# jgrss/cultionet

Hardware: AMD Instinct MI355X
Metric: train_chips_per_sec (higher is better)
Workload: dtype f32

## Files before the change

### cultionet_amd/csrc/cn_conv.hip

```cpp
#include "cn_common.h"
#include "cn_conv_geom.h"
#include "cn_profile.h"

#include <cstdlib>

#define KC 8

static int cn_reduce_slices(const CnConvGeom& g, hipStream_t stream);

template <int TN, int TM>
__device__ __forceinline__ void cn_igemm_epilogue(const CnConvGeom& g, const f32x16 (&acc)[TN][TM],
                                                  const bool (&pix_ok)[TM], const int (&out_off)[TM], int co_base,
                                                  int half, int grp, int split, int b,
                                                  const float* __restrict__ bias, float* __restrict__ y) {
  const int HWout = g.Hout * g.Wout;
  const bool sliced = g.slice_stride != 0;
  float* yb = sliced ? g.part + (long)(grp * g.splits + split) * g.slice_stride + (long)b * g.Cout * HWout
                     : y + (long)b * g.ybs;
  const bool first = split == 0;
#pragma unroll
  for (int tn = 0; tn < TN; ++tn) {
#pragma unroll
    for (int r = 0; r < 16; ++r) {
      const int co = co_base + tn * 32 + (r & 3) + 8 * (r >> 2) + 4 * half;
// ... 549 lines not shown
  if ((long)g.Cin * g.Hin * g.Win * 4 >= (1L << 31) || (long)(max_taps > 0 ? max_taps : 1) * g.Kpad * g.Npad * 4 >= (1L << 31))
    return CN_ERR_ARG;
  const size_t lds = (size_t)(g.tap_lds_off + 3 * CN_MAX_TAPS + 1) * sizeof(float);
  if (lds > 160 * 1024) return CN_ERR_LDS;
  static bool attr_set = false;
  if (!attr_set) {
    (void)hipFuncSetAttribute((const void*)cn_conv_igemm_kernel<WAVES_N, TN, NI_T>,
                              hipFuncAttributeMaxDynamicSharedMemorySize, 160 * 1024);
    attr_set = true;
  }
  g.grid_x = total_tiles;
  g.grid_y = (g.Cout + NT - 1) / NT;
  g.splits = splits < 1 ? 1 : splits;
  dim3 grid(cn_xcd_grid((long)g.grid_x * g.grid_y * g.splits));
  cn_prof_name("cn_conv_igemm_kernel<%d, %d, %d>", WAVES_N, TN, NI_T);
  cn_prof_desc("igemm_dw<%d,%d,%d> G%d B%d %d->%d %dx%d->%dx%d taps%d cls%d is%d os%d grid%dx%dx%d", WAVES_N, TN, NI_T,
               g.G, g.B, g.Cin, g.Cout, g.Hin, g.Win, g.Hout, g.Wout, max_taps, g.ncls, g.is, g.os, total_tiles,
               (g.Cout + NT - 1) / NT, splits);
  cn_prof_bytes(4.0 * g.G * ((double)g.B * g.Cin * g.Hin * g.Win + (double)g.B * g.Cout * g.Hout * g.Wout / (g.shared_y ? g.G : 1) +
                             (double)(max_taps > 0 ? max_taps : 1) * g.Cin * g.Cout));
  cn_prof_before(stream);
  CN_LAUNCH((cn_conv_igemm_kernel<WAVES_N, TN, NI_T>), grid, dim3(256), lds, stream, g);
  cn_prof_after(stream, NT == 128 ? 0 : 1, flops);
  const int rrc = cn_reduce_slices(g, stream);
  return rrc != CN_OK ? rrc : cn_check_launch();
}

struct CnPlan {
  int total_tiles, max_plane, max_vplane, max_taps;
  int max_rplane, max_absdx;
  double flops;
};

static CnPlan cn_plan(CnConvGeom& g, int MT) {
  CnPlan p = {0, 0, 0, 0, 0, 0, 0.0};
  for (int c = 0; c < g.ncls; ++c) {
    CnConvClass& k = g.cls[c];
    const int Mimg = k.Hg * k.Wg;
    int rows_g = (MT + k.Wg - 2) / k.Wg + 1;
    if (rows_g > k.Hg) rows_g = k.Hg;
    k.min_dy = 0; k.min_dx = 0;
    int max_dy = 0, max_dx = 0;
    for (int t = 0; t < k.ntaps; ++t) {
      if (t == 0 || k.dy[t] < k.min_dy) k.min_dy = k.dy[t];
      if (t == 0 || k.dx[t] < k.min_dx) k.min_dx = k.dx[t];
      if (t == 0 || k.dy[t] > max_dy) max_dy = k.dy[t];
      if (t == 0 || k.dx[t] > max_dx) max_dx = k.dx[t];
    }
    const int rows = (rows_g - 1) * g.is + (max_dy - k.min_dy) + 1;
    k.pitch = (k.Wg - 1) * g.is + (max_dx - k.min_dx) + 1;
    k.plane = rows * k.pitch;
    k.vplane = (rows * g.Win + (max_dx - k.min_dx) + 4 + 3) / 4 * 4;
    k.rows = rows;
    {
      const int rpitch = (g.Win + 3) / 4 * 4 + 4;
      if ((rows + 1) * rpitch + 4 > p.max_rplane) p.max_rplane = (rows + 1) * rpitch + 4;
    }
    if (-k.min_dx > p.max_absdx) p.max_absdx = -k.min_dx;
    if (max_dx > p.max_absdx) p.max_absdx = max_dx;
    k.tiles_per_img = (Mimg + MT - 1) / MT;
    k.block_begin = p.total_tiles;
    p.total_tiles += g.B * k.tiles_per_img;
    if (k.plane > p.max_plane) p.max_plane = k.plane;
    if (k.vplane > p.max_vplane) p.max_vplane = k.vplane;
    if (k.ntaps > p.max_taps) p.max_taps = k.ntaps;
    p.flops += 2.0 * g.B * Mimg * (double)g.Cout * g.Cin * k.ntaps;
  }
  g.interleave = 0;
  if (g.ncls > 1 && g.want_interleave) {
    bool same = true;
    for (int c = 1; c < g.ncls; ++c) same = same && g.cls[c].tiles_per_img == g.cls[0].tiles_per_img;
    g.interleave = same ? 1 : 0;
  }
  return p;
}

struct CnChoice { int cfg, splits, cps; double cost; };

static double cn_launch_cost(long blocks, int cps, double mt_units, int splits, double out_elems) {
  const double F = 273.0, R = 170.0;
  const double c1 = 36.7 + 0.614 * mt_units, c2 = 30.0 + 1.19 * mt_units;
  const long full = blocks / 512, rem = blocks % 512;
  double c = full * (F + cps * c2);
  if (rem > 0) c += F + cps * (rem > 256 ? c2 : c1);
  if (splits > 1) c += R + out_elems * 4.0 * (2.0 * splits + 1.0) / 8.0e6 * (128.0 / 7.5);
  return c;
}

static thread_local float* g_conv_ws;
static thread_local long g_conv_ws_floats;

static CnChoice cn_choose(const CnConvGeom& g0, const int* mts, int ncfg, int NT, bool allow_split) {
  const int nchunks = (g0.Cin + KC - 1) / KC;
  const int ny = (g0.Cout + NT - 1) / NT;
  const int G = g0.G > 0 ? g0.G : 1;
  const double out_elems = (double)g0.B * g0.Cout * g0.Hout * g0.Wout * (g0.shared_y ? 1 : G);
  CnChoice best = {0, 1, nchunks > 0 ? nchunks : 1, 1e300};
  int forced = 0;
  {
    static const char* dbg = getenv("CN_DBG_SPLITS");
    if (dbg) forced = atoi(dbg) < 1 ? 1 : atoi(dbg);
  }
  long ws_cap = 32;
  if (g_conv_ws != nullptr) {
    const long stride = ((long)g0.B * g0.Cout * g0.Hout * g0.Wout + 3) / 4 * 4;
    ws_cap = g_conv_ws_floats / (stride * G);
  }
  int forced_cfg = -1;
  {
    static const char* dbgc = getenv("CN_DBG_CFG");
    if (dbgc) forced_cfg = atoi(dbgc);
  }
  for (int i = 0; i < ncfg; ++i) {
    if (forced_cfg >= 0 && i != (forced_cfg < ncfg ? forced_cfg : ncfg - 1)) continue;
    CnConvGeom gi = g0;
    const CnPlan p = cn_plan(gi, mts[i]);
    if (p.total_tiles <= 0) continue;
    const long base = (long)p.total_tiles * ny;
    int max_splits = (allow_split && p.max_taps > 0 && nchunks >= 4) ? nchunks / 2 : 1;
    if (max_splits > 32) max_splits = 32;
    if (max_splits > ws_cap) max_splits = ws_cap < 1 ? 1 : (int)ws_cap;
    const double taps = p.total_tiles > 0 ? p.flops / (2.0 * g0.Cout * g0.Cin * (double)mts[i] * p.total_tiles) : 9.0;
    const double chunk_units = (double)mts[i] * NT / 128.0 * (taps < 9.0 ? taps : 9.0) / 9.0;
    for (int sp = 1; sp <= max_splits; ++sp) {
      if (forced && sp != (forced > max_splits ? max_splits : forced)) continue;
      const int cps = (nchunks + sp - 1) / sp;
      const int splits = (nchunks + cps - 1) / cps;
      if (splits != sp && !forced) continue;
      const double cost = cn_launch_cost(base * splits, cps, chunk_units, splits, out_elems);
      if (cost < best.cost * (i == best.cfg ? 1.0 : 0.98)) best = {i, splits, cps, cost};
    }
  }
  return best;
}


#include <mutex>
#include <unordered_map>
namespace {
struct CnWs { float* p; long n; };
std::mutex g_ws_mu;
std::unordered_map<void*, CnWs> g_ws_by_stream;
}

extern "C" int cn_conv_set_workspace(void* stream, float* ws, long ws_floats) {
  if (ws != nullptr && ((reinterpret_cast<uintptr_t>(ws) & 15) || ws_floats < 0)) return CN_ERR_ARG;
  std::lock_guard<std::mutex> lk(g_ws_mu);
  if (ws == nullptr) g_ws_by_stream.erase(stream);
  else g_ws_by_stream[stream] = {ws, ws_floats};
  return CN_OK;
}

static void cn_bind_ws(void* stream) {
  std::lock_guard<std::mutex> lk(g_ws_mu);
  auto it = g_ws_by_stream.find(stream);
  if (it == g_ws_by_stream.end()) { g_conv_ws = nullptr; g_conv_ws_floats = 0; }
  else { g_conv_ws = it->second.p; g_conv_ws_floats = it->second.n; }
}

struct CnReduceArgs {
  const float* part;
  long slice_stride;
  int nsum;
  int ngrp;
  float* y[CN_MAX_GROUPS];
  const float* bias[CN_MAX_GROUPS * CN_MAX_GROUPS];
  int nbias;
  long ybs;
  int B, Cout, HW, accumulate;
};

__global__ __launch_bounds__(256) void cn_conv_reduce_kernel(const CnReduceArgs a) {
  const long n = (long)a.Cout * a.HW;
  const int b = blockIdx.y, gi = blockIdx.z;
  const float* p0 = a.part + (long)gi * a.nsum * a.slice_stride + (long)b * n;
  float* yb = a.y[gi] + (long)b * a.ybs;
  for (long i = (blockIdx.x * 256L + threadIdx.x) * 4; i < n; i += (long)gridDim.x * 1024) {
    if (i + 3 < n && (n & 3) == 0 && (a.ybs & 3) == 0 && (reinterpret_cast<uintptr_t>(yb) & 15) == 0) {
      f32x4 s = *reinterpret_cast<const f32x4*>(p0 + i);
      for (int k = 1; k < a.nsum; ++k) s += *reinterpret_cast<const f32x4*>(p0 + (long)k * a.slice_stride + i);
#pragma unroll
      for (int e = 0; e < 4; ++e) {
        const int c = (int)((i + e) / a.HW);
        for (int j = 0; j < a.nbias; ++j)
          if (a.bias[gi * CN_MAX_GROUPS + j] != nullptr) s[e] += a.bias[gi * CN_MAX_GROUPS + j][c];
      }
      f32x4* d = reinterpret_cast<f32x4*>(yb + i);
      *d = a.accumulate ? *d + s : s;
    } else {
      for (long e = i; e < n && e < i + 4; ++e) {
        float s = p0[e];
        for (int k = 1; k < a.nsum; ++k) s += p0[(long)k * a.slice_stride + e];
        const int c = (int)(e / a.HW);
        for (int j = 0; j < a.nbias; ++j)
          if (a.bias[gi * CN_MAX_GROUPS + j] != nullptr) s += a.bias[gi * CN_MAX_GROUPS + j][c];
        yb[e] = a.accumulate ? yb[e] + s : s;
      }
    }
  }
}

static int cn_finish_split(CnConvGeom& g, const CnPlan& p, int splits, int cps, float* y, hipStream_t stream) {
  (void)y;
  const int nchunks = (g.Cin + KC - 1) / KC;
  g.chunks_per_split = cps > 0 ? cps : (nchunks > 0 ? nchunks : 1);
  if (p.max_taps == 0) g.chunks_per_split = nchunks > 0 ? nchunks : 1;
  g.splits = splits < 1 ? 1 : splits;
  g.atomic_out = g.splits > 1 || (g.G > 1 && g.shared_y);
  g.part = nullptr;
  g.slice_stride = 0;
  if (g.atomic_out) {
    const long stride = ((long)g.B * g.Cout * g.Hout * g.Wout + 3) / 4 * 4;
    if (g_conv_ws != nullptr && stride * g.G * g.splits <= g_conv_ws_floats) {
      g.part = g_conv_ws;
      g.slice_stride = stride;
      return CN_OK;
    }
  }
  if (g.atomic_out && !g.accumulate) {
    const int ny = g.shared_y ? 1 : g.G;
    for (int i = 0; i < ny; ++i)
      if (hipMemsetAsync(g.gy[i], 0, sizeof(float) * (size_t)g.B * g.Cout * g.Hout * g.Wout, stream) != hipSuccess)
        return CN_ERR_LAUNCH;
  }
  return CN_OK;
}

static int cn_reduce_slices(const CnConvGeom& g, hipStream_t stream) {
  if (g.slice_stride == 0) return CN_OK;
  CnReduceArgs a = {};
  a.part = g.part;
  a.slice_stride = g.slice_stride;
  a.ybs = g.ybs; a.B = g.B; a.Cout = g.Cout; a.HW = g.Hout * g.Wout; a.accumulate = g.accumulate;
  if (g.shared_y) {
    a.nsum = g.G * g.splits; a.ngrp = 1; a.y[0] = g.gy[0]; a.nbias = g.G;
    for (int j = 0; j < g.G; ++j) a.bias[j] = g.gbias[j];
  } else {
    a.nsum = g.splits; a.ngrp = g.G; a.nbias = 1;
    for (int i = 0; i < g.G; ++i) { a.y[i] = g.gy[i]; a.bias[i * CN_MAX_GROUPS] = g.gbias[i]; }
  }
  const long n = (long)g.Cout * a.HW;
  long bx = (n + 1023) / 1024;
  if (bx > 1024) bx = 1024;
  CN_LAUNCH(cn_conv_reduce_kernel, dim3((unsigned)bx, g.B, a.ngrp), dim3(256), 0, stream, a);
  return cn_check_launch();
}

template <int WAVES_N, int TN, int TM>
static int cn_launch_vec_cfg(const float* x, const float* wp, const float* bias, float* y, CnConvGeom& g, int splits,
                             int cps, hipStream_t stream) {
  constexpr int MT = (4 / WAVES_N) * TM * 32;
  const CnPlan p = cn_plan(g, MT);
  if (p.total_tiles <= 0) return CN_OK;
  const int rp = g.odd_planes ? 3
                 : (p.max_rplane <= 4096 && p.max_absdx <= 4) ? (g.Win % 4 == 0 ? 1 : (g.Win % 2 == 0 ? 2 : 0)) : 0;
  const int img = (rp == 1 || rp == 2) ? p.max_rplane : p.max_vplane;
  g.w_lds_off = KC * 1024 * (img <= 1024 ? 1 : (img <= 2048 ? 2 : 4)) + (rp == 3 ? 16 : 0);
  const int rc = cn_finish_split(g, p, splits, cps, y, stream);
  if (rc != CN_OK) return rc;
#define CN_GO(NV_, RP_) \
  return cn_launch_igemm_v<WAVES_N, TN, TM, NV_, RP_>(x, wp, bias, y, g, p.total_tiles, p.max_taps, splits, p.flops, stream)
  if (rp == 1) {
    if (img <= 1024) CN_GO(1, 1);
    if (img <= 2048) CN_GO(2, 1);
    CN_GO(4, 1);
  }
  if (rp == 2) {
    if (img <= 1024) CN_GO(1, 2);
    if (img <= 2048) CN_GO(2, 2);
    CN_GO(4, 2);
  }
  if (rp == 3) {
    if (img <= 1024) CN_GO(1, 3);
    if (img <= 2048) CN_GO(2, 3);
    CN_GO(4, 3);
  }
  if (img <= 1024) CN_GO(1, 0);
  if (img <= 2048) CN_GO(2, 0);
  CN_GO(4, 0);
#undef CN_GO
}

template <int WAVES_N, int TN>
static int cn_launch_dword_cfg(const float* x, const float* wp, const float* bias, float* y, CnConvGeom& g,
                               int splits, int cps, hipStream_t stream) {
  constexpr int MT = (4 / WAVES_N) * 64;
  const CnPlan p = cn_plan(g, MT);
  if (p.total_tiles <= 0) return CN_OK;
  if (p.max_plane > 12 * 256) return CN_ERR_LDS;
  g.w_lds_off = (KC * p.max_plane + 3) / 4 * 4;
  const int rc = cn_finish_split(g, p, splits, cps, y, stream);
  if (rc != CN_OK) return rc;
  if (p.max_plane <= 3 * 256)
    return cn_launch_igemm_t<WAVES_N, TN, 3>(x, wp, bias, y, g, p.total_tiles, p.max_taps, splits, p.flops, stream);
  if (p.max_plane <= 6 * 256)
    return cn_launch_igemm_t<WAVES_N, TN, 6>(x, wp, bias, y, g, p.total_tiles, p.max_taps, splits, p.flops, stream);
  return cn_launch_igemm_t<WAVES_N, TN, 12>(x, wp, bias, y, g, p.total_tiles, p.max_taps, splits, p.flops, stream);
}

struct CnGemm1x1 {
  int B, Cin, Cout, HW, Kpad, Npad, tiles_per_img, grid_x, grid_y, accumulate;
  long xbs, ybs;
};
#define KC1 32

template <int TM>
__global__ __launch_bounds__(256) void cn_conv1x1_kernel(const float* __restrict__ x, const float* __restrict__ wp,
                                                        const float* __restrict__ bias, float* __restrict__ y,
                                                        const CnGemm1x1 g) {
  constexpr int MT = TM * 32, NT = 128;
  constexpr int NA = KC1 * NT / 4 / 256;
  constexpr int NB = (KC1 * MT / 4 + 255) / 256;
  __shared__ __attribute__((aligned(16))) float a_lds[KC1 * NT];
  __shared__ __attribute__((aligned(16))) float b_lds[KC1 * MT];
  int bx, by, bz;
  if (!cn_xcd_block(g.grid_x, g.grid_y, g.grid_x * g.grid_y, bx, by, bz)) return;
  const int tid = threadIdx.x, lane = tid & 63, wn = tid >> 6;
  const int half = lane >> 5, l31 = lane & 31;
  const int b = bx / g.tiles_per_img;
  const int p0 = (bx - b * g.tiles_per_img) * MT;
  const int n0 = by * NT;
  const float* xb = x + (long)b * g.xbs;

  f32x16 acc[TM];
#pragma unroll
  for (int tm = 0; tm < TM; ++tm)
#pragma unroll
    for (int r = 0; r < 16; ++r) acc[tm][r] = 0.f;

  f32x4 ra[NA], rb[NB];
  const f32x4 zero4 = {0.f, 0.f, 0.f, 0.f};
#define CN_G1_PREFETCH(c0_)                                                                          \
  {                                                                                                  \
    const int c0 = (c0_);                                                                            \
    _Pragma("unroll") for (int k = 0; k < NA; ++k) {                                                 \
      const int i = tid + k * 256, row = i / (NT / 4), c4 = i - row * (NT / 4);                      \
      ra[k] = (c0 + row) < g.Kpad                                                                    \
                  ? *reinterpret_cast<const f32x4*>(wp + (long)(c0 + row) * g.Npad + n0 + c4 * 4)    \
                  : zero4;                                                                           \
    }                                                                                                \
    _Pragma("unroll") for (int k = 0; k < NB; ++k) {                                                 \
      const int i = tid + k * 256, row = i / (MT / 4), q = i - row * (MT / 4);                       \
      const int p = p0 + q * 4;                                                                      \
      rb[k] = (i < KC1 * MT / 4 && (c0 + row) < g.Cin && p < g.HW)                                   \
                  ? *reinterpret_cast<const f32x4*>(xb + (long)(c0 + row) * g.HW + p)                \
                  : zero4;                                                                           \
    }                                                                                                \
  }
  const int nchunks = (g.Cin + KC1 - 1) / KC1;
  CN_G1_PREFETCH(0);
  for (int ch = 0; ch < nchunks; ++ch) {
    __syncthreads();
#pragma unroll
    for (int k = 0; k < NA; ++k) *reinterpret_cast<f32x4*>(a_lds + (tid + k * 256) * 4) = ra[k];
#pragma unroll
    for (int k = 0; k < NB; ++k)
      if (tid + k * 256 < KC1 * MT / 4) *reinterpret_cast<f32x4*>(b_lds + (tid + k * 256) * 4) = rb[k];
    __syncthreads();
    if (ch + 1 < nchunks) CN_G1_PREFETCH((ch + 1) * KC1);
    const float* ap = a_lds + half * NT + wn * 32 + l31;
    const float* bp = b_lds + half * MT + l31;
#pragma unroll
    for (int k2 = 0; k2 < KC1 / 2; ++k2) {
      const float av = ap[k2 * 2 * NT];
#pragma unroll
      for (int tm = 0; tm < TM; ++tm)
        acc[tm] = __builtin_amdgcn_mfma_f32_32x32x2f32(av, bp[k2 * 2 * MT + tm * 32], acc[tm], 0, 0, 0);
    }
  }
#undef CN_G1_PREFETCH
  float* yb = y + (long)b * g.ybs;
#pragma unroll
  for (int r = 0; r < 16; ++r) {
    const int co = n0 + wn * 32 + (r & 3) + 8 * (r >> 2) + 4 * half;
    if (co < g.Cout) {
      const float bv = bias != nullptr ? bias[co] : 0.f;
#pragma unroll
      for (int tm = 0; tm < TM; ++tm) {
        const int p = p0 + tm * 32 + l31;
        if (p < g.HW) {
          float* dst = yb + (long)co * g.HW + p;
          const float v = acc[tm][r] + bv;
          *dst = g.accumulate ? *dst + v : v;
        }
      }
    }
  }
}

static int cn_conv1x1_launch(const float* x, long xbs, const float* wp, const float* bias, float* y, long ybs, int B,
                             int Cin, int HW, int Cout, int accumulate, hipStream_t stream) {
  if ((HW & 3) || (xbs & 3) || (reinterpret_cast<uintptr_t>(x) & 15)) return CN_ERR_ARG;
  CnGemm1x1 g = {};
  g.B = B; g.Cin = Cin; g.Cout = Cout; g.HW = HW; g.xbs = xbs; g.ybs = ybs; g.accumulate = accumulate;
  g.Kpad = cn_conv_kpad(Cin);
  g.Npad = cn_conv_npad(Cout);
  if (cn_pick_nt(Cout) != 128) return CN_ERR_ARG;
  g.grid_y = (Cout + 127) / 128;
  const long t160 = (long)B * ((HW + 159) / 160) * g.grid_y, t128 = (long)B * ((HW + 127) / 128) * g.grid_y;
  const bool use160 = ((t160 + 511) / 512) * 160 <= ((t128 + 511) / 512) * 128;
  const long blocks = use160 ? t160 : t128;
  if (blocks < 256) return CN_ERR_ARG;
  g.tiles_per_img = use160 ? (HW + 159) / 160 : (HW + 127) / 128;
  g.grid_x = B * g.tiles_per_img;
  const double flops = 2.0 * B * HW * (double)Cout * Cin;
  cn_prof_name("cn_conv1x1_kernel<%d>", use160 ? 5 : 4);
  cn_prof_desc("gemm1x1<%d> B%d %d->%d HW%d grid%dx%d", use160 ? 5 : 4, B, Cin, Cout, HW, g.grid_x, g.grid_y);
  cn_prof_before(stream);
  if (use160)
    CN_LAUNCH((cn_conv1x1_kernel<5>), dim3(cn_xcd_grid(blocks)), dim3(256), 0, stream, x, wp, bias, y, g);
  else
    CN_LAUNCH((cn_conv1x1_kernel<4>), dim3(cn_xcd_grid(blocks)), dim3(256), 0, stream, x, wp, bias, y, g);
  cn_prof_after(stream, 0, flops);
  return cn_check_launch();
}

#include <functional>
static int g_autotune = 0;
static std::unordered_map<uint64_t, CnChoice> g_tuned;
static std::mutex g_tune_mu;

extern "C" int cn_conv_set_autotune(int on) {
  std::lock_guard<std::mutex> lk(g_tune_mu);
  g_autotune = on ? 1 : 0;
  if (!on) g_tuned.clear();
  return CN_OK;
}

static uint64_t cn_tune_key(const CnConvGeom& g, bool vec, int nt, bool allow_split) {
  uint64_t h = 1469598103934665603ull;
  auto mix = [&](long v) { h = (h ^ (uint64_t)v) * 1099511628211ull; };
  mix(g.B); mix(g.Cin); mix(g.Hin); mix(g.Win); mix(g.Cout); mix(g.Hout); mix(g.Wout); mix(g.is); mix(g.os);
  mix(g.ncls); mix(g.G); mix(g.shared_y); mix(vec); mix(nt); mix(allow_split); mix(g_conv_ws != nullptr);
  for (int c = 0; c < g.ncls; ++c) {
    const CnConvClass& k = g.cls[c];
    mix(k.Hg); mix(k.Wg); mix(k.ntaps); mix(k.grp);
    for (int t = 0; t < k.ntaps; ++t) { mix(k.dy[t]); mix(k.dx[t]); }
  }
  return h;
}

static CnChoice cn_autotune(const CnConvGeom& g, const int* mts, int ncfg, int nt, bool allow_split,
                            const CnChoice& model, const std::function<int(const CnChoice&, CnConvGeom&)>& run,
                            hipStream_t stream) {
  static const int split_set[] = {1, 2, 3, 4, 6, 8, 12, 16, 24, 32};
  const int nchunks = (g.Cin + KC - 1) / KC;
  const int ny = (g.Cout + nt - 1) / nt;
  long ws_cap = 32;
  if (g_conv_ws != nullptr) {
    const long stride = ((long)g.B * g.Cout * g.Hout * g.Wout + 3) / 4 * 4;
    ws_cap = g_conv_ws_floats / (stride * (g.G > 0 ? g.G : 1));
  }
  hipEvent_t e0, e1;
  if (hipEventCreate(&e0) != hipSuccess || hipEventCreate(&e1) != hipSuccess) return model;
  CnChoice best = model;
  float best_ms = 1e30f;
  for (int i = 0; i < ncfg; ++i) {
    CnConvGeom gi = g;
    const CnPlan p = cn_plan(gi, mts[i]);
    if (p.total_tiles <= 0) continue;
    int max_splits = (allow_split && p.max_taps > 0 && nchunks >= 4) ? nchunks / 2 : 1;
    if (max_splits > 32) max_splits = 32;
    if (max_splits > ws_cap) max_splits = ws_cap < 1 ? 1 : (int)ws_cap;
    for (int sp : split_set) {
      if (sp > max_splits) break;
      const int cps = (nchunks + sp - 1) / sp;
      const int splits = (nchunks + cps - 1) / cps;
      if (splits != sp) continue;
      if ((long)p.total_tiles * ny * splits > 8192) continue;
      const CnChoice c = {i, splits, cps, 0.0};
      float ms = 0.f;
      bool ok = true;
      for (int rep = 0; rep < 2 && ok; ++rep) {
        CnConvGeom gg = g;
        ok = hipEventRecord(e0, stream) == hipSuccess && run(c, gg) == CN_OK &&
             hipEventRecord(e1, stream) == hipSuccess && hipEventSynchronize(e1) == hipSuccess &&
             hipEventElapsedTime(&ms, e0, e1) == hipSuccess;
      }
      if (ok && ms < best_ms) { best_ms = ms; best = c; }
    }
  }
  (void)hipEventDestroy(e0);
  (void)hipEventDestroy(e1);
  return best;
}

int cn_conv_igemm_launch(CnConvGeom& g, hipStream_t stream) {
  if (g.ncls < 1 || g.ncls > CN_MAX_CLASSES || g.B <= 0 || g.G < 1) return g.B <= 0 ? CN_OK : CN_ERR_ARG;
  g.splits = 1;
  const float* x = g.gx[0]; const float* wp = g.gwp[0]; const float* bias = g.gbias[0]; float* y = g.gy[0];
  g.Kpad = cn_conv_kpad(g.Cin);
  g.Npad = cn_conv_npad(g.Cout);
  const int nt = cn_pick_nt(g.Cout);
  const bool dense_out = g.ybs == (long)g.Cout * g.Hout * g.Wout;
  const bool ws_fits = g_conv_ws != nullptr &&
                       (((long)g.B * g.Cout * g.Hout * g.Wout + 3) / 4 * 4) * g.G * 32 <= g_conv_ws_floats;
  const bool allow_split = dense_out || g.accumulate || ws_fits;
  if (g.G > 1 && g.shared_y && !allow_split) return CN_ERR_ARG;
  const int hw4 = (int)(((long)g.Hin * g.Win) % 4);
  g.odd_planes = (hw4 == 1 && !(g.is > 1 && (long)g.Hin * g.Win > 4096)) ? 1 : 0;
  bool vec = (hw4 == 0 || g.odd_planes) && (g.xbs % 4 == 0);
  if (g.is > 1 && (long)g.Hin * g.Win > 4096) vec = false;
  if ((long)g.Cin * g.Hin * g.Win * 4 >= (1L << 31) || (long)CN_MAX_TAPS * cn_conv_kpad(g.Cin) * g.Npad * 4 >= (1L << 31))
    return CN_ERR_ARG;
  for (int i = 0; i < g.G; ++i) vec = vec && ((reinterpret_cast<uintptr_t>(g.gx[i]) & 15) == 0);
  if (vec) {
    CnConvGeom t = g;
    vec = cn_plan(t, 256).max_vplane <= 4 * 1024;
  }
  static const int mts128[3] = {128, 96, 160};
  static const int mts128d[1] = {128};
  static const int mts256[1] = {256};
  const int* mts = nt == 128 ? (vec ? mts128 : mts128d) : mts256;
  const int ncfg = (nt == 128 && vec) ? 3 : 1;
  auto run = [&](const CnChoice& c, CnConvGeom& gg) -> int {
    if (nt == 128) {
      if (vec) {
        switch (c.cfg) {
          case 1: return cn_launch_vec_cfg<4, 1, 3>(x, wp, bias, y, gg, c.splits, c.cps, stream);
          case 2: return cn_launch_vec_cfg<4, 1, 5>(x, wp, bias, y, gg, c.splits, c.cps, stream);
          default: return cn_launch_vec_cfg<2, 2, 2>(x, wp, bias, y, gg, c.splits, c.cps, stream);
        }
      }
      return cn_launch_dword_cfg<2, 2>(x, wp, bias, y, gg, c.splits, c.cps, stream);
    }
    int rc;
    if (nt == 64) {
      if (vec) return cn_launch_vec_cfg<1, 2, 2>(x, wp, bias, y, gg, c.splits, c.cps, stream);
      rc = cn_launch_dword_cfg<1, 2>(x, wp, bias, y, gg, c.splits, c.cps, stream);
    } else {
      if (vec) return cn_launch_vec_cfg<1, 1, 2>(x, wp, bias, y, gg, c.splits, c.cps, stream);
      rc = cn_launch_dword_cfg<1, 1>(x, wp, bias, y, gg, c.splits, c.cps, stream);
    }
    if (rc == CN_ERR_LDS) {
      CnConvGeom g2 = gg;
      rc = cn_launch_dword_cfg<2, 2>(x, wp, bias, y, g2, c.splits, c.cps, stream);
    }
    return rc;
  };
  CnChoice c = cn_choose(g, mts, ncfg, nt, allow_split);
  if (g_autotune) {
    std::lock_guard<std::mutex> lk(g_tune_mu);
    const uint64_t key = cn_tune_key(g, vec, nt, allow_split);
    auto it = g_tuned.find(key);
    if (it != g_tuned.end()) {
      c = it->second;
    } else if (!g.accumulate && !cn_prof_on()) {
      c = cn_autotune(g, mts, ncfg, nt, allow_split, c, run, stream);
      g_tuned.emplace(key, c);
    }
  }
  return run(c, g);
}

static int cn_set_groups(CnConvGeom& g, int G, const float* const* xs, const float* const* wps,
                         const float* const* biases, float* const* ys) {
  if (G < 1 || G > CN_MAX_GROUPS) return CN_ERR_ARG;
  g.G = G;
  int same = 0;
  for (int i = 0; i < G; ++i) {
    g.gx[i] = xs[i]; g.gwp[i] = wps[i]; g.gbias[i] = biases ? biases[i] : nullptr; g.gy[i] = ys[i];
    if (ys[i] == ys[0]) ++same;
  }
  if (same != G && same != 1) return CN_ERR_ARG;
  for (int i = 1; i < G && same == 1; ++i)
    for (int j = 1; j < i; ++j)
      if (ys[i] == ys[j]) return CN_ERR_ARG;
  g.shared_y = (G > 1 && same == G) ? 1 : 0;
  g.has_bias = 0;
  for (int i = 0; i < G; ++i) g.has_bias |= g.gbias[i] != nullptr;
  return CN_OK;
}

static int cn_gather_conv_g(int G, const float* const* xs, long xbs, const float* const* wps,
                            const float* const* biases, float* const* ys, long ybs, int B, int Cin, int Hin,
                            int Win, int Cout, int Hout, int Wout, int KH, int KW, int stride, const int* pads,
                            const int* dils, int accumulate, hipStream_t stream) {
  if (KH * KW > CN_MAX_TAPS || stride < 1) return CN_ERR_ARG;
  if (Hout <= 0 || Wout <= 0) return CN_OK;
  if (G == 1 && KH == 1 && KW == 1 && stride == 1 && pads[0] == 0 && Hout == Hin && Wout == Win) {
    const int r1 = cn_conv1x1_launch(xs[0], xbs, wps[0], biases ? biases[0] : nullptr, ys[0], ybs, B, Cin, Hin * Win,
                                     Cout, accumulate, stream);
    if (r1 != CN_ERR_ARG) return r1;
  }
  CnConvGeom g = {};
  const int rc = cn_set_groups(g, G, xs, wps, biases, ys);
  if (rc != CN_OK) return rc;
  g.B = B; g.Cin = Cin; g.Hin = Hin; g.Win = Win; g.Cout = Cout; g.Hout = Hout; g.Wout = Wout;
  g.xbs = xbs; g.ybs = ybs; g.is = stride; g.os = 1;
  g.ncls = G;
  for (int i = 0; i < G; ++i) {
    if (dils[i] < 1) return CN_ERR_ARG;
    CnConvClass& k = g.cls[i];
    k.grp = i;
    k.Hg = Hout; k.Wg = Wout; k.oy0 = 0; k.ox0 = 0;
    k.ntaps = cn_gather_taps(KH, KW, pads[i], dils[i], k.dy, k.dx, k.wt);
  }
  g.accumulate = accumulate;
  return cn_conv_igemm_launch(g, stream);
}

static int cn_gather_conv(const float* x, long xbs, const float* wp, const float* bias, float* y, long ybs, int B,
                          int Cin, int Hin, int Win, int Cout, int Hout, int Wout, int KH, int KW, int stride,
                          int pad, int dil, int accumulate, hipStream_t stream) {
  return cn_gather_conv_g(1, &x, xbs, &wp, &bias, &y, ybs, B, Cin, Hin, Win, Cout, Hout, Wout, KH, KW, stride, &pad,
                          &dil, accumulate, stream);
}

extern "C" int cn_conv2d_fwd_f32(const float* x, long xbs, const float* wp, const float* bias, float* y,
                                 long ybs, int B, int Cin, int Hin, int Win, int Cout, int KH, int KW,
                                 int stride, int pad, int dil, int accumulate, void* stream) {
  cn_bind_ws(stream);
  if (stride < 1) return CN_ERR_ARG;
  const int Hout = cn_conv_out(Hin, KH, stride, pad, dil);
  const int Wout = cn_conv_out(Win, KW, stride, pad, dil);
  return cn_gather_conv(x, xbs, wp, bias, y, ybs, B, Cin, Hin, Win, Cout, Hout, Wout, KH, KW, stride, pad, dil,
                        accumulate, (hipStream_t)stream);
}

static int cn_scatter_conv_g(int G, const float* const* srcs, long sbs, const float* const* wps,
                             const float* const* biases, float* const* outs, long obs, int B, int Csrc, int Hs,
                             int Ws, int Cdst, int Ho, int Wo, const int* khs, const int* kws, int stride,
                             const int* pads, const int* dils, int accumulate, hipStream_t stream) {
  if (stride < 1 || G * stride * stride > CN_MAX_CLASSES) return CN_ERR_ARG;
  for (int i = 0; i < G; ++i)
    if (khs[i] * kws[i] > CN_MAX_TAPS || khs[i] < 1 || kws[i] < 1) return CN_ERR_ARG;
  if (G == 1 && khs[0] == 1 && kws[0] == 1 && stride == 1 && pads[0] == 0 && Ho == Hs && Wo == Ws) {
    const int r1 = cn_conv1x1_launch(srcs[0], sbs, wps[0], biases ? biases[0] : nullptr, outs[0], obs, B, Csrc,
                                     Hs * Ws, Cdst, accumulate, stream);
    if (r1 != CN_ERR_ARG) return r1;
  }
  CnConvGeom g = {};
  const int rc = cn_set_groups(g, G, srcs, wps, biases, outs);
  if (rc != CN_OK) return rc;
  g.B = B; g.Cin = Csrc; g.Hin = Hs; g.Win = Ws; g.Cout = Cdst; g.Hout = Ho; g.Wout = Wo;
  g.xbs = sbs; g.ybs = obs; g.is = 1; g.os = stride;
  g.accumulate = accumulate;
  int nc = 0;
  for (int gi = 0; gi < G; ++gi) {
    const int pad = pads[gi], dil = dils[gi], KH = khs[gi], KW = kws[gi];
    if (dil < 1) return CN_ERR_ARG;
    for (int py = 0; py < stride; ++py)
      for (int px = 0; px < stride; ++px) {
        CnConvClass& k = g.cls[nc];
        k.grp = gi;
        k.Hg = cn_parity_extent(Ho, py, stride);
        k.Wg = cn_parity_extent(Wo, px, stride);
        if (k.Hg <= 0 || k.Wg <= 0) continue;
        k.oy0 = py; k.ox0 = px;
        k.ntaps = cn_parity_taps(py, px, KH, KW, stride, pad, dil, k.dy, k.dx, k.wt);
        ++nc;
      }
  }
  g.ncls = nc;
  if (nc == 0) return CN_OK;
  cn_sort_heavy_first(g.cls, nc);
  g.want_interleave = stride > 1 ? 1 : 0;
  return cn_conv_igemm_launch(g, stream);
}

static int cn_scatter_conv(const float* src, long sbs, const float* wp, const float* bias, float* out, long obs,
                           int B, int Csrc, int Hs, int Ws, int Cdst, int Ho, int Wo, int KH, int KW,
                           int stride, int pad, int dil, int accumulate, hipStream_t stream) {
  return cn_scatter_conv_g(1, &src, sbs, &wp, &bias, &out, obs, B, Csrc, Hs, Ws, Cdst, Ho, Wo, &KH, &KW, stride, &pad,
                           &dil, accumulate, stream);
}

extern "C" int cn_conv2d_bwd_data_f32(const float* dy, long dybs, const float* wp_t, float* dx, long dxbs,
                                      int B, int Cin, int Hin, int Win, int Cout, int KH, int KW, int stride,
                                      int pad, int dil, int accumulate, void* stream) {
  cn_bind_ws(stream);
  if (stride < 1) return CN_ERR_ARG;
  const int Hout = cn_conv_out(Hin, KH, stride, pad, dil);
  const int Wout = cn_conv_out(Win, KW, stride, pad, dil);
  return cn_scatter_conv(dy, dybs, wp_t, nullptr, dx, dxbs, B, Cout, Hout, Wout, Cin, Hin, Win, KH, KW, stride,
                         pad, dil, accumulate, (hipStream_t)stream);
}

extern "C" int cn_conv2d_fwd_grouped_f32(int G, const float* const* xs, long xbs, const float* const* wps,
                                         const float* const* biases, float* const* ys, long ybs, int B, int Cin,
                                         int Hin, int Win, int Cout, int KH, int KW, int stride, const int* pads,
                                         const int* dils, int accumulate, void* stream) {
  cn_bind_ws(stream);
  if (G < 1 || G > CN_MAX_GROUPS) return CN_ERR_ARG;
  if (stride < 1) return CN_ERR_ARG;
  const int Hout = cn_conv_out(Hin, KH, stride, pads[0], dils[0]);
  const int Wout = cn_conv_out(Win, KW, stride, pads[0], dils[0]);
  for (int i = 1; i < G; ++i)
    if (cn_conv_out(Hin, KH, stride, pads[i], dils[i]) != Hout ||
        cn_conv_out(Win, KW, stride, pads[i], dils[i]) != Wout)
      return CN_ERR_ARG;
  return cn_gather_conv_g(G, xs, xbs, wps, biases, ys, ybs, B, Cin, Hin, Win, Cout, Hout, Wout, KH, KW, stride,
                          pads, dils, accumulate, (hipStream_t)stream);
}

extern "C" int cn_conv2d_bwd_data_grouped_f32(int G, const float* const* dys, long dybs, const float* const* wps_t,
                                              float* const* dxs, long dxbs, int B, int Cin, int Hin, int Win,
                                              int Cout, const int* khs, const int* kws, int stride, const int* pads,
                                              const int* dils, int accumulate, void* stream) {
  cn_bind_ws(stream);
  if (G < 1 || G > CN_MAX_GROUPS) return CN_ERR_ARG;
  if (stride < 1) return CN_ERR_ARG;
  const int Hout = cn_conv_out(Hin, khs[0], stride, pads[0], dils[0]);
  const int Wout = cn_conv_out(Win, kws[0], stride, pads[0], dils[0]);
  for (int i = 1; i < G; ++i)
    if (cn_conv_out(Hin, khs[i], stride, pads[i], dils[i]) != Hout ||
        cn_conv_out(Win, kws[i], stride, pads[i], dils[i]) != Wout)
      return CN_ERR_ARG;
  return cn_scatter_conv_g(G, dys, dybs, wps_t, nullptr, dxs, dxbs, B, Cout, Hout, Wout, Cin, Hin, Win, khs, kws,
                           stride, pads, dils, accumulate, (hipStream_t)stream);
}

extern "C" int cn_conv_transpose2d_fwd_f32(const float* x, long xbs, const float* wp, const float* bias,
                                           float* y, long ybs, int B, int Cin, int Hin, int Win, int Cout,
                                           int KH, int KW, int stride, int pad, int out_pad, int accumulate,
                                           void* stream) {
  cn_bind_ws(stream);
// ... 70 lines not shown
```

Before: 385.0.

## Rewrite 1x1 conv GEMM with direct global-to-LDS DMA multi-stage pipeline

Replaces the register-staged 1x1 conv GEMM with a templated kernel that copies weight and activation tiles straight into LDS through global_load_lds, using an NST-deep buffer ring synchronised by explicit vmcnt waits and barriers. It adds odd-HW and dword-aligned staging variants plus smaller tile configurations chosen by a cost heuristic, so shapes that earlier returned an argument error (unaligned HW, Cout not suited to 128-wide tiles, too few blocks) now run on the GEMM path. The goal is to hide global load latency, drop the register round-trip, and cover more layers. In exchange it relies on hand-written inline waitcnt asm and dynamic LDS sizing, and the odd-HW path uses skewed indexing that is easy to get wrong.

```diff
diff --git a/cultionet_amd/csrc/cn_conv.hip b/cultionet_amd/csrc/cn_conv.hip
--- a/cultionet_amd/csrc/cn_conv.hip
+++ b/cultionet_amd/csrc/cn_conv.hip
@@ -875,73 +875,134 @@
   int B, Cin, Cout, HW, Kpad, Npad, tiles_per_img, grid_x, grid_y, accumulate;
   long xbs, ybs;
 };
-#define KC1 32
-
-template <int TM>
-__global__ __launch_bounds__(256) void cn_conv1x1_kernel(const float* __restrict__ x, const float* __restrict__ wp,
-                                                        const float* __restrict__ bias, float* __restrict__ y,
-                                                        const CnGemm1x1 g) {
-  constexpr int MT = TM * 32, NT = 128;
-  constexpr int NA = KC1 * NT / 4 / 256;
-  constexpr int NB = (KC1 * MT / 4 + 255) / 256;
-  __shared__ __attribute__((aligned(16))) float a_lds[KC1 * NT];
-  __shared__ __attribute__((aligned(16))) float b_lds[KC1 * MT];
+#define CN_G1_ALIGNED 0
+#define CN_G1_ODD 1
+#define CN_G1_DWORD 2
+
+typedef __attribute__((address_space(3))) void* cn_g1_lds_ptr;
+typedef const __attribute__((address_space(1))) void* cn_g1_gbl_ptr;
+static __device__ float cn_g1_zero[256];
+
+template <int BYTES>
+__device__ __forceinline__ void cn_g1_glds(const float* src, float* lds_wave_base) {
+  if constexpr (BYTES == 16)
+    __builtin_amdgcn_global_load_lds((cn_g1_gbl_ptr)src, (cn_g1_lds_ptr)lds_wave_base, 16, 0, 0);
+  else
+    __builtin_amdgcn_global_load_lds((cn_g1_gbl_ptr)src, (cn_g1_lds_ptr)lds_wave_base, 4, 0, 0);
+}
+
+template <int WN, int WM, int TM, int KCH, int STG, int NST>
+struct CnG1Cfg {
+  static constexpr int NW = WN * WM, NT = WN * 32, MT = WM * TM * 32;
+  static constexpr int VB = STG == CN_G1_DWORD ? 4 : 16;
+  static constexpr int MTP = MT + (STG == CN_G1_ODD ? 4 : 0);
+  static constexpr int BPI = VB == 16 ? 256 : 64;
+  static constexpr int NBI = (KCH * MTP + BPI - 1) / BPI;
+  static constexpr int BIMG = NBI * BPI;
+  static constexpr int AIMG = KCH * NT;
+  static constexpr size_t LDS = sizeof(float) * NST * (AIMG + BIMG);
+};
+
+template <int WN, int WM, int TM, int KCH, int STG, int NST>
+__global__ __launch_bounds__(64 * WN * WM) void cn_gemm1x1_kernel(const float* __restrict__ x,
+                                                                  const float* __restrict__ wp,
+                                                                  const float* __restrict__ bias,
+                                                                  float* __restrict__ y, const CnGemm1x1 g) {
+  using C = CnG1Cfg<WN, WM, TM, KCH, STG, NST>;
+  constexpr int NW = C::NW, NT = C::NT, MT = C::MT, VB = C::VB, MTP = C::MTP, BPI = C::BPI, NBI = C::NBI;
+  constexpr int BIMG = C::BIMG, AIMG = C::AIMG;
+  constexpr int NA = AIMG / 256 / NW;
+  constexpr int NBW = (NBI + NW - 1) / NW;
+  constexpr bool ODD = STG == CN_G1_ODD;
+  static_assert(AIMG % (256 * NW) == 0, "a weight chunk is a whole number of DMA instructions per wave");
+  static_assert(STG != CN_G1_DWORD || (MT & (MT - 1)) == 0, "the dword variant decodes pixels with shifts");
+  constexpr int INFL = (NST - 2) * (NA + NBI / NW);
+  static_assert(NST >= 2 && INFL < 64, "vmcnt is a 6-bit counter");
+  extern __shared__ __attribute__((aligned(16))) float smem[];
+  float* a_lds = smem;
+  float* b_lds = smem + NST * AIMG;
+
   int bx, by, bz;
   if (!cn_xcd_block(g.grid_x, g.grid_y, g.grid_x * g.grid_y, bx, by, bz)) return;
-  const int tid = threadIdx.x, lane = tid & 63, wn = tid >> 6;
+  const int tid = threadIdx.x, lane = tid & 63;
+  const int wid = __builtin_amdgcn_readfirstlane(tid >> 6);
   const int half = lane >> 5, l31 = lane & 31;
+  const int wn = wid % WN, wm = wid / WN;
   const int b = bx / g.tiles_per_img;
   const int p0 = (bx - b * g.tiles_per_img) * MT;
+  const float* xb = x + (long)b * g.xbs;
+  const float* zero16 = cn_g1_zero + 4 * lane;
+  const float* zerob = cn_g1_zero + (VB == 16 ? 4 : 1) * lane;
+  const int nch = (g.Cin + KCH - 1) / KCH;
+  const long img = (long)g.Cin * g.HW;
+
   const int n0 = by * NT;
-  const float* xb = x + (long)b * g.xbs;
+  auto stage_a = [&](int c0, int buf) {
+    float* dst = a_lds + buf * AIMG;
+#pragma unroll
+    for (int k = 0; k < NA; ++k) {
+      const int inst = wid + NW * k;
+      const int p = inst * 64 + lane;
+      const int row = c0 + p / (NT / 4), c4 = p % (NT / 4);
+      const float* src = row < g.Kpad ? wp + (long)row * g.Npad + n0 + 4 * c4 : zero16;
+      cn_g1_glds<16>(src, dst + inst * 256);
+    }
+  };
+  auto stage_b = [&](int c0, int buf) {
+    float* dst = b_lds + buf * BIMG;
+#pragma unroll
+    for (int k = 0; k < NBW; ++k) {
+      const int inst = wid + NW * k;
+      if (NBI % NW == 0 || inst < NBI) {
+        const int e = inst * BPI + (VB == 16 ? 4 : 1) * lane;
+        const int r = e / MTP, row = c0 + r;
+        const int pix = p0 + e % MTP - (ODD ? (row & 3) : 0);
+        const long f = (long)row * g.HW + pix;
+        bool ok = r < KCH && row < g.Cin && pix < g.HW;
+        if (ODD) ok = ok && f + 3 < img;
+        const float* src = ok ? xb + f : zerob;
+        cn_g1_glds<VB>(src, dst + inst * BPI);
+      }
+    }
+  };
 
   f32x16 acc[TM];
 #pragma unroll
   for (int tm = 0; tm < TM; ++tm)
 #pragma unroll
     for (int r = 0; r < 16; ++r) acc[tm][r] = 0.f;
-
-  f32x4 ra[NA], rb[NB];
-  const f32x4 zero4 = {0.f, 0.f, 0.f, 0.f};
-#define CN_G1_PREFETCH(c0_)                                                                          \
-  {                                                                                                  \
-    const int c0 = (c0_);                                                                            \
-    _Pragma("unroll") for (int k = 0; k < NA; ++k) {                                                 \
-      const int i = tid + k * 256, row = i / (NT / 4), c4 = i - row * (NT / 4);                      \
-      ra[k] = (c0 + row) < g.Kpad                                                                    \
-                  ? *reinterpret_cast<const f32x4*>(wp + (long)(c0 + row) * g.Npad + n0 + c4 * 4)    \
-                  : zero4;                                                                           \
-    }                                                                                                \
-    _Pragma("unroll") for (int k = 0; k < NB; ++k) {                                                 \
-      const int i = tid + k * 256, row = i / (MT / 4), q = i - row * (MT / 4);                       \
-      const int p = p0 + q * 4;                                                                      \
-      rb[k] = (i < KC1 * MT / 4 && (c0 + row) < g.Cin && p < g.HW)                                   \
-                  ? *reinterpret_cast<const f32x4*>(xb + (long)(c0 + row) * g.HW + p)                \
-                  : zero4;                                                                           \
-    }                                                                                                \
-  }
-  const int nchunks = (g.Cin + KC1 - 1) / KC1;
-  CN_G1_PREFETCH(0);
-  for (int ch = 0; ch < nchunks; ++ch) {
-    __syncthreads();
-#pragma unroll
-    for (int k = 0; k < NA; ++k) *reinterpret_cast<f32x4*>(a_lds + (tid + k * 256) * 4) = ra[k];
-#pragma unroll
-    for (int k = 0; k < NB; ++k)
-      if (tid + k * 256 < KC1 * MT / 4) *reinterpret_cast<f32x4*>(b_lds + (tid + k * 256) * 4) = rb[k];
-    __syncthreads();
-    if (ch + 1 < nchunks) CN_G1_PREFETCH((ch + 1) * KC1);
-    const float* ap = a_lds + half * NT + wn * 32 + l31;
-    const float* bp = b_lds + half * MT + l31;
-#pragma unroll
-    for (int k2 = 0; k2 < KC1 / 2; ++k2) {
+  auto compute = [&](int buf) {
+    const float* ap = a_lds + buf * AIMG + half * NT + wn * 32 + l31;
+    const float* bp = b_lds + buf * BIMG + half * (MTP + (ODD ? 1 : 0)) + wm * (TM * 32) + l31;
+#pragma unroll
+    for (int k2 = 0; k2 < KCH / 2; ++k2) {
       const float av = ap[k2 * 2 * NT];
 #pragma unroll
       for (int tm = 0; tm < TM; ++tm)
-        acc[tm] = __builtin_amdgcn_mfma_f32_32x32x2f32(av, bp[k2 * 2 * MT + tm * 32], acc[tm], 0, 0, 0);
-    }
-  }
-#undef CN_G1_PREFETCH
+        acc[tm] = __builtin_amdgcn_mfma_f32_32x32x2f32(av, bp[k2 * 2 * MTP + (ODD ? (2 * k2) & 3 : 0) + tm * 32], acc[tm],
+                                                       0, 0, 0);
+    }
+  };
+#pragma unroll
+  for (int s = 0; s < NST - 1; ++s)
+    if (s < nch) {
+      stage_a(s * KCH, s);
+      stage_b(s * KCH, s);
+    }
+  int buf = 0, nbuf = NST - 1;
+  for (int ch = 0; ch < nch; ++ch) {
+    if (ch + NST - 1 <= nch)
+      asm volatile("s_waitcnt vmcnt(%0) lgkmcnt(0)\n\ts_barrier" ::"n"(INFL) : "memory");
+    else
+      asm volatile("s_waitcnt vmcnt(0) lgkmcnt(0)\n\ts_barrier" ::: "memory");
+    if (ch + NST - 1 < nch) {
+      stage_a((ch + NST - 1) * KCH, nbuf);
+      stage_b((ch + NST - 1) * KCH, nbuf);
+    }
+    compute(buf);
+    buf = buf + 1 == NST ? 0 : buf + 1;
+    nbuf = nbuf + 1 == NST ? 0 : nbuf + 1;
+  }
   float* yb = y + (long)b * g.ybs;
 #pragma unroll
   for (int r = 0; r < 16; ++r) {
@@ -950,7 +1011,7 @@
       const float bv = bias != nullptr ? bias[co] : 0.f;
 #pragma unroll
       for (int tm = 0; tm < TM; ++tm) {
-        const int p = p0 + tm * 32 + l31;
+        const int p = p0 + wm * (TM * 32) + tm * 32 + l31;
         if (p < g.HW) {
           float* dst = yb + (long)co * g.HW + p;
           const float v = acc[tm][r] + bv;
@@ -961,31 +1022,66 @@
   }
 }
 
+template <int WN, int WM, int TM, int KCH, int STG, int NST>
+static int cn_gemm1x1_go(const float* x, const float* wp, const float* bias, float* y, CnGemm1x1& g,
+                         hipStream_t stream) {
+  using C = CnG1Cfg<WN, WM, TM, KCH, STG, NST>;
+  g.tiles_per_img = (g.HW + C::MT - 1) / C::MT;
+  g.grid_x = g.B * g.tiles_per_img;
+  g.grid_y = (g.Cout + C::NT - 1) / C::NT;
+  constexpr size_t lds = C::LDS;
+  static_assert(lds <= 160 * 1024, "LDS of one CU");
+  static bool attr_set = false;
+  if (!attr_set) {
+    (void)hipFuncSetAttribute((const void*)cn_gemm1x1_kernel<WN, WM, TM, KCH, STG, NST>,
+                              hipFuncAttributeMaxDynamicSharedMemorySize, 160 * 1024);
+    attr_set = true;
+  }
+  const double flops = 2.0 * g.B * g.HW * (double)g.Cout * g.Cin;
+  cn_prof_name("cn_gemm1x1_kernel<%d, %d, %d, %d, %d, %d>", WN, WM, TM, KCH, STG, NST);
+  cn_prof_desc("gemm1x1<%dx%d,k%dx%d,%s> B%d %d->%d HW%d grid%dx%d", C::NT, C::MT, KCH, NST,
+               STG == CN_G1_ALIGNED ? "v16" : (STG == CN_G1_ODD ? "odd16" : "v4"), g.B, g.Cin, g.Cout, g.HW, g.grid_x,
+               g.grid_y);
+  cn_prof_before(stream);
+  CN_LAUNCH((cn_gemm1x1_kernel<WN, WM, TM, KCH, STG, NST>), dim3(cn_xcd_grid((long)g.grid_x * g.grid_y)),
+            dim3(64 * WN * WM), lds, stream, x, wp, bias, y, g);
+  cn_prof_after(stream, 0, flops);
+  return cn_check_launch();
+}
+
 static int cn_conv1x1_launch(const float* x, long xbs, const float* wp, const float* bias, float* y, long ybs, int B,
                              int Cin, int HW, int Cout, int accumulate, hipStream_t stream) {
-  if ((HW & 3) || (xbs & 3) || (reinterpret_cast<uintptr_t>(x) & 15)) return CN_ERR_ARG;
+  if (B <= 0 || Cin <= 0 || Cout <= 0 || HW <= 0) return CN_ERR_ARG;
+  if (reinterpret_cast<uintptr_t>(wp) & 15) return CN_ERR_ARG;
   CnGemm1x1 g = {};
   g.B = B; g.Cin = Cin; g.Cout = Cout; g.HW = HW; g.xbs = xbs; g.ybs = ybs; g.accumulate = accumulate;
   g.Kpad = cn_conv_kpad(Cin);
   g.Npad = cn_conv_npad(Cout);
-  if (cn_pick_nt(Cout) != 128) return CN_ERR_ARG;
-  g.grid_y = (Cout + 127) / 128;
-  const long t160 = (long)B * ((HW + 159) / 160) * g.grid_y, t128 = (long)B * ((HW + 127) / 128) * g.grid_y;
-  const bool use160 = ((t160 + 511) / 512) * 160 <= ((t128 + 511) / 512) * 128;
-  const long blocks = use160 ? t160 : t128;
-  if (blocks < 256) return CN_ERR_ARG;
-  g.tiles_per_img = use160 ? (HW + 159) / 160 : (HW + 127) / 128;
-  g.grid_x = B * g.tiles_per_img;
-  const double flops = 2.0 * B * HW * (double)Cout * Cin;
-  cn_prof_name("cn_conv1x1_kernel<%d>", use160 ? 5 : 4);
-  cn_prof_desc("gemm1x1<%d> B%d %d->%d HW%d grid%dx%d", use160 ? 5 : 4, B, Cin, Cout, HW, g.grid_x, g.grid_y);
-  cn_prof_before(stream);
-  if (use160)
-    CN_LAUNCH((cn_conv1x1_kernel<5>), dim3(cn_xcd_grid(blocks)), dim3(256), 0, stream, x, wp, bias, y, g);
-  else
-    CN_LAUNCH((cn_conv1x1_kernel<4>), dim3(cn_xcd_grid(blocks)), dim3(256), 0, stream, x, wp, bias, y, g);
-  cn_prof_after(stream, 0, flops);
-  return cn_check_launch();
+  const bool img16 = !(xbs & 3) && !(reinterpret_cast<uintptr_t>(x) & 15);
+  const int stg = (img16 && (HW & 3) == 0) ? CN_G1_ALIGNED
+                  : (img16 && (HW & 3) == 1 && (Cin & 3) == 0) ? CN_G1_ODD : CN_G1_DWORD;
+  const int nt = cn_pick_nt(Cout);
+  auto blocks = [&](int ntile, int mtile) {
+    return (long)B * ((HW + mtile - 1) / mtile) * ((Cout + ntile - 1) / ntile);
+  };
+#define CN_G1_GO(WN_, WM_, TM_, KCH_, NST_)                                                                        \
+  return stg == CN_G1_ALIGNED ? cn_gemm1x1_go<WN_, WM_, TM_, KCH_, CN_G1_ALIGNED, NST_>(x, wp, bias, y, g, stream) \
+         : stg == CN_G1_ODD   ? cn_gemm1x1_go<WN_, WM_, TM_, KCH_, CN_G1_ODD, NST_>(x, wp, bias, y, g, stream)     \
+                              : cn_gemm1x1_go<WN_, WM_, TM_, KCH_, CN_G1_DWORD, NST_>(x, wp, bias, y, g, stream)
+  if (nt == 128 && stg == CN_G1_ALIGNED) {
+    const long t160 = blocks(128, 160), t128 = blocks(128, 128);
+    const bool use160 = ((t160 + 511) / 512) * 160 <= ((t128 + 511) / 512) * 128;
+    if (use160 && t160 >= 256) return cn_gemm1x1_go<4, 1, 5, 32, CN_G1_ALIGNED, 2>(x, wp, bias, y, g, stream);
+    if (!use160 && t128 >= 256) return cn_gemm1x1_go<4, 1, 4, 32, CN_G1_ALIGNED, 2>(x, wp, bias, y, g, stream);
+  }
+  if (nt == 128 && stg == CN_G1_ODD && blocks(128, 128) >= 256)
+    return cn_gemm1x1_go<4, 1, 4, 32, CN_G1_ODD, 2>(x, wp, bias, y, g, stream);
+  auto cost = [&](int ntile, int mtile) { return ((blocks(ntile, mtile) + 255) / 256) * (ntile + mtile); };
+  const long c64 = nt >= 64 ? cost(64, 64) : (1L << 60), c32x64 = cost(32, 64), c32 = cost(32, 32);
+  if (c64 <= c32x64 && c64 <= c32) { CN_G1_GO(2, 2, 1, 32, 3); }
+  if (c32x64 <= c32) { CN_G1_GO(1, 2, 1, 32, 4); }
+  CN_G1_GO(1, 1, 1, 32, 4);
+#undef CN_G1_GO
 }
 
 #include <functional>
```

Measured after the change: 392.6, median of 6. 1.02x the previous value.
